# pierluigiferrari/ssd_keras

Hardware: AMD Instinct MI355X
Metric: images/sec SSD300 fwd+decode @batch32 (higher is better)
Workload: dtype f32 (decode, threshold, TF-style f32 NMS, top-k); bf16 conv backbone; 1 GPU; SSD300 VGG-16 inference (mode='inference': forward + DecodeDetections), 21 classes, batch 32 per GPU, conf 0.01 / NMS 0.45 / top-200, random-init weights, synthetic 300x300x3 uint8-range images; per_gpu_batch=32, global_batch=32, conv_dtype=bf16, parallelism=replicas x1, launch=hip_graph (forward + DecodeDetections captured once, replayed per step), decode_stream=same stream; DecodeDetections reads the head outputs directly (no y_pred in HBM)

## Files before the change

ssd_keras_amd/csrc/ssdhip_decode.hip:

```cpp
#include <hip/hip_runtime.h>
#include <stdint.h>
#include <stdlib.h>

#include "ssdhip.h"
#include "ssdhip_math.h"
#include "ssdhip_tile.h"
#include "ssdhip_heads.h"
#include "ssdhip_decode64.h"

#ifdef SSDHIP_PROFILE
__device__ unsigned long long g_prof[64];
#define PROF_DECL long long _pt = clock64(); long long _pa[12] = {0, 0, 0, 0, 0, 0, 0, 0, 0, 0, 0, 0};
#define PROF_MARK(i) { const long long _t = clock64(); _pa[i] += _t - _pt; _pt = _t; }
#define PROF_FLUSH(base) if (threadIdx.x == 0) { for (int _i = 0; _i < 12; ++_i) if (_pa[_i]) atomicAdd(&g_prof[(base) + _i], (unsigned long long)_pa[_i]); }
extern "C" int ssdhip_profile_read(unsigned long long* host_out, int reset) {
    if (hipMemcpyFromSymbol(host_out, HIP_SYMBOL(g_prof), sizeof(g_prof)) != hipSuccess) return -1;
    if (reset) { unsigned long long z[64] = {0}; if (hipMemcpyToSymbol(HIP_SYMBOL(g_prof), z, sizeof(z)) != hipSuccess) return -1; }
    return 0;
}
#else
#define PROF_DECL
#define PROF_MARK(i)
#define PROF_FLUSH(base)
#endif

namespace ssdhip {

constexpr int IDX_BITS = 20;
constexpr u32 IDX_MASK = (1u << IDX_BITS) - 1u;
constexpr int DIGIT_BITS = 13;
constexpr int NBINS = 1 << DIGIT_BITS;
constexpr int NMS_BIN_SHIFT = 14;
constexpr int NMS_NBINS = 4096;
#ifndef SSDHIP_MAX_CHUNK
#define SSDHIP_MAX_CHUNK 512
#endif
#ifndef SSDHIP_NMS_MINWAVES
#define SSDHIP_NMS_MINWAVES 3
#endif
constexpr int MAX_CHUNK = SSDHIP_MAX_CHUNK;
constexpr int KEPT_LDS = 256;
constexpr int KC_KEYS = 9216;
constexpr int TOPK_SORT_MAX = 4096;

struct DecodeParams {
    int B, N, C, L, G;
    int class_agnostic, semantics, coords, border;
    int thr_inclusive;
    float thr_eff;
    u32 thr_key;
    int iou_f32;
    int fast_ok;
    int px_f32;
    int no_nms;
    float filter_kE;
    double iou_thresh, img_w, img_h;
    int top_k, cap, cap_store, out_rows, sorted;
    int no_dma;
};

template <int SHIFT, int NB>
__device__ __forceinline__ int bin_of(u32 skey, u32 thr_key) {
    const u32 v = skey >> SHIFT, base = thr_key >> SHIFT;
    if (v <= base) return 0;
    const u32 d = v - base;
    return d > (u32)(NB - 1) ? NB - 1 : (int)d;
}

template <int SEM>
__device__ __forceinline__ float decode_center(float off, float var, float a_wh, float a_c) {
    if (SEM == SSDHIP_SEM_KERAS) return (off * var) * a_wh + a_c;
    if (SEM == SSDHIP_SEM_DEBUG) return (off * a_wh) * var + a_c;
    return off * (var * a_wh) + a_c;
}

__device__ __forceinline__ void scan_tile_body(const float* tile, int* wave_cnt, const DecodeParams& p, const int b, const int a0,
                                               const int na, float4* __restrict__ boxes, u64* __restrict__ cand,
                                               int* __restrict__ cand_count, unsigned short* __restrict__ cls_out) {
    const int TA = blockDim.x;
    const int L = p.L;
    const int tid = threadIdx.x;
    const int lane = tid & 63, wave = tid >> 6, nwaves = TA >> 6;
    PROF_DECL
    PROF_MARK(0)

    const bool active = tid < na;
    const float* row = tile + (size_t)tid * L;
    const int C = p.C;

    int fast_cls = 0;
    float fast_conf = 0.f;
    if (active) {
        const float o0 = row[C], o1 = row[C + 1], o2 = row[C + 2], o3 = row[C + 3];
        const float a_0 = row[C + 4], a_1 = row[C + 5], a_2 = row[C + 6], a_3 = row[C + 7];
        const float v0 = row[C + 8], v1 = row[C + 9], v2 = row[C + 10], v3 = row[C + 11];
        float4 box;
        if (p.coords == SSDHIP_CENTROIDS) {
            float cx, cy;
            if (p.semantics == SSDHIP_SEM_KERAS) {
                cx = decode_center<SSDHIP_SEM_KERAS>(o0, v0, a_2, a_0);
                cy = decode_center<SSDHIP_SEM_KERAS>(o1, v1, a_3, a_1);
            } else if (p.semantics == SSDHIP_SEM_DEBUG) {
                cx = decode_center<SSDHIP_SEM_DEBUG>(o0, v0, a_2, a_0);
                cy = decode_center<SSDHIP_SEM_DEBUG>(o1, v1, a_3, a_1);
            } else {
                cx = decode_center<SSDHIP_SEM_NUMPY>(o0, v0, a_2, a_0);
                cy = decode_center<SSDHIP_SEM_NUMPY>(o1, v1, a_3, a_1);
            }
            const float w = det_expf(o2 * v2) * a_2;
            const float h = det_expf(o3 * v3) * a_3;
            const float hw = w / 2.0f, hh = h / 2.0f;
            box = make_float4(cx - hw, cy - hh, cx + hw, cy + hh);
        } else if (p.coords == SSDHIP_MINMAX) {
            const float aw = a_1 - a_0, ah = a_3 - a_2;
            const float t0 = (o0 * v0) * aw + a_0, t1 = (o1 * v1) * aw + a_1;
            const float t2 = (o2 * v2) * ah + a_2, t3 = (o3 * v3) * ah + a_3;
            box = make_float4(t0, t2, t1, t3);
        } else {
            const float aw = a_2 - a_0, ah = a_3 - a_1;
            box = make_float4((o0 * v0) * aw + a_0, (o1 * v1) * ah + a_1, (o2 * v2) * aw + a_2, (o3 * v3) * ah + a_3);
        }
        boxes[(size_t)b * p.N + a0 + tid] = box;
        if (p.class_agnostic) {
            float best = row[0];
            int bi = 0;
            for (int c = 1; c < C; ++c) {
                const float s = row[c];
                if (s > best) { best = s; bi = c; }
            }
            for (int c = 0; c < C; ++c) if (row[c] != row[c]) { best = row[c]; bi = c; break; }
            fast_cls = bi;
            fast_conf = best;
            cls_out[(size_t)b * p.N + a0 + tid] = (unsigned short)bi;
        }
    }
    PROF_MARK(1)

    const int G = p.G;
    const float t = p.thr_eff;
    const bool incl = p.thr_inclusive != 0;
    const bool fast_pred = active && (fast_cls != 0) && (incl ? (fast_conf >= t) : (fast_conf > t));
    for (int gb = 0; gb < G; gb += 64) {
        const int ng = min(64, G - gb);
        int mycnt = 0;
        if (p.class_agnostic) {
            mycnt = __popcll(__ballot(fast_pred));
        } else {
            const float* sc = row + gb + 1;
            for (int j0 = 0; j0 < ng; j0 += 8) {
                float s8[8];
#pragma unroll
                for (int u = 0; u < 8; ++u) s8[u] = sc[min(j0 + u, ng - 1)];
#pragma unroll
                for (int u = 0; u < 8; ++u) {
                    const bool pr = active && (j0 + u < ng) && (incl ? (s8[u] >= t) : (s8[u] > t));
                    const int cnt = __popcll(__ballot(pr));
                    mycnt = lane == j0 + u ? cnt : mycnt;
                }
            }
        }
        if (lane < ng) wave_cnt[wave * G + gb + lane] = mycnt;
    }
    __syncthreads();
    PROF_MARK(2)
    for (int g = tid; g < G; g += TA) {
        int tot = 0;
        for (int w = 0; w < nwaves; ++w) tot += wave_cnt[w * G + g];
        int base = 0;
        if (tot) base = atomicAdd(&cand_count[b * G + g], tot);
        for (int w = 0; w < nwaves; ++w) {
            const int c = wave_cnt[w * G + g];
            wave_cnt[w * G + g] = base;
            base += c;
        }
    }
    __syncthreads();
    PROF_MARK(3)
    const u32 inv_idx = IDX_MASK - (u32)(a0 + tid);
    for (int gb = 0; gb < G; gb += 64) {
        const int ng = min(64, G - gb);
        const int mybase = lane < ng ? wave_cnt[wave * G + gb + lane] : 0;
        const float* sc = row + gb + 1;
        for (int j0 = 0; j0 < ng; j0 += 8) {
            float s8[8];
#pragma unroll
            for (int u = 0; u < 8; ++u) s8[u] = p.class_agnostic ? fast_conf : sc[min(j0 + u, ng - 1)];
#pragma unroll
            for (int u = 0; u < 8; ++u) {
                const int j = j0 + u;
                const float s = s8[u];
                const bool pr = (j < ng) && (p.class_agnostic ? fast_pred : (active && (incl ? (s >= t) : (s > t))));
                const u64 m = __ballot(pr);
                if (m == 0) continue;
                const int base_j = __builtin_amdgcn_readlane(mybase, j);
                if (pr) {
                    const int slot = base_j + (int)__builtin_amdgcn_mbcnt_hi((u32)(m >> 32), __builtin_amdgcn_mbcnt_lo((u32)m, 0u));
                    cand[((size_t)b * G + gb + j) * p.N + slot] = ((u64)float_key(s) << IDX_BITS) | inv_idx;
                }
            }
        }
    }
    PROF_MARK(4)
    PROF_FLUSH(16)
}

__global__ __launch_bounds__(256) void scan_kernel(const float* __restrict__ y, DecodeParams p,
                                                   float4* __restrict__ boxes, u64* __restrict__ cand,
                                                   int* __restrict__ cand_count, unsigned short* __restrict__ cls_out) {
    extern __shared__ __attribute__((aligned(16))) unsigned char smem_raw[];
    const int TA = blockDim.x;
    const int b = blockIdx.y;
    const int a0 = blockIdx.x * TA;
    const int na = min(TA, p.N - a0);
    const float* tile;
    const size_t total_bytes = (size_t)gridDim.y * p.N * (size_t)p.L * sizeof(float);
    if (!((uintptr_t)y & 15) && !(((size_t)p.N * p.L) & 3) && !((TA * p.L) & 3) && total_bytes < 0x7fffff00ull && !(TA & 63) && !p.no_dma) {
        const int lane = threadIdx.x & 63, wave = __builtin_amdgcn_readfirstlane((int)threadIdx.x >> 6);
        const u32 lds0 = (u32)(uintptr_t)(__attribute__((address_space(3))) unsigned char*)smem_raw;
        const i32x4 rs = tile_rsrc(y, (u32)total_bytes);
        const u32 off = (u32)(((size_t)b * p.N + a0) * (size_t)p.L * sizeof(float));
        const int nch = (na * p.L + 3) >> 2;
        for (int q0 = wave * 64; q0 < nch; q0 += TA) {
            const int q = q0 + lane;
            tile_dma16(q < nch ? off + (u32)q * 16u : TILE_OOB, rs, lds0 + (u32)q0 * 16u);
        }
        asm volatile("s_waitcnt vmcnt(0)" ::: "memory");
        tile = reinterpret_cast<const float*>(smem_raw);
    } else {
        tile = tile_copy_f32(reinterpret_cast<float*>(smem_raw), y + ((size_t)b * p.N + a0) * (size_t)p.L, na * p.L, threadIdx.x, TA);
    }
    int* wave_cnt = reinterpret_cast<int*>(smem_raw + (((size_t)TA * p.L + 4) * sizeof(float) + 15) / 16 * 16);
    __syncthreads();
    scan_tile_body(tile, wave_cnt, p, b, a0, na, boxes, cand, cand_count, cls_out);
}

constexpr int SW_WAVES = 4, SW_CW = 32, SW_PITCH = SW_CW + 1;
__global__ __launch_bounds__(SW_WAVES * 64) void scan_wide_kernel(const float* __restrict__ y, DecodeParams p, float4* __restrict__ boxes,
                                                                  u64* __restrict__ cand, int* __restrict__ cand_count) {
    __shared__ float win_all[SW_WAVES][64 * SW_PITCH];
    const int tid = threadIdx.x, lane = tid & 63, wave = tid >> 6;
    const int b = blockIdx.y;
    const int a0 = ((int)blockIdx.x * SW_WAVES + wave) * 64;
    if (a0 >= p.N) return;
    const int na = min(64, p.N - a0);
    float* win = win_all[wave];
    const int L = p.L, C = p.C, G = p.G;
    const float* src = y + ((size_t)b * p.N + a0) * (size_t)L;
    const float t = p.thr_eff;
    const bool incl = p.thr_inclusive != 0;
    const bool active = lane < na;
    const u32 inv_idx = IDX_MASK - (u32)(a0 + lane);
    const int nwin = (L + SW_CW - 1) / SW_CW;
    for (int wi = nwin - 1; wi >= 0; --wi) {
        const int c_hi = L - (nwin - 1 - wi) * SW_CW, c_lo = max(0, c_hi - SW_CW), cw = c_hi - c_lo;
        {
            const int c = lane & 31, rh = lane >> 5;
#pragma unroll
            for (int r0 = 0; r0 < 64; r0 += 16) {
                float v[8];
#pragma unroll
                for (int u = 0; u < 8; ++u) {
                    const int r = r0 + 2 * u + rh;
                    v[u] = (r < na && c < cw) ? src[(size_t)r * L + c_lo + c] : 0.f;
                }
#pragma unroll
                for (int u = 0; u < 8; ++u) win[(r0 + 2 * u + rh) * SW_PITCH + c] = v[u];
            }
        }
        __builtin_amdgcn_fence(__ATOMIC_RELEASE, "workgroup");
        __builtin_amdgcn_wave_barrier();
        const float* row = win + lane * SW_PITCH;
        if (wi == nwin - 1 && active) {
            const float* q = row + (cw - 12);
            const float o0 = q[0], o1 = q[1], o2 = q[2], o3 = q[3];
            const float a_0 = q[4], a_1 = q[5], a_2 = q[6], a_3 = q[7];
            const float v0 = q[8], v1 = q[9], v2 = q[10], v3 = q[11];
            float4 box;
            if (p.coords == SSDHIP_CENTROIDS) {
                float cx, cy;
                if (p.semantics == SSDHIP_SEM_KERAS) {
                    cx = decode_center<SSDHIP_SEM_KERAS>(o0, v0, a_2, a_0);
                    cy = decode_center<SSDHIP_SEM_KERAS>(o1, v1, a_3, a_1);
                } else if (p.semantics == SSDHIP_SEM_DEBUG) {
                    cx = decode_center<SSDHIP_SEM_DEBUG>(o0, v0, a_2, a_0);
                    cy = decode_center<SSDHIP_SEM_DEBUG>(o1, v1, a_3, a_1);
                } else {
                    cx = decode_center<SSDHIP_SEM_NUMPY>(o0, v0, a_2, a_0);
                    cy = decode_center<SSDHIP_SEM_NUMPY>(o1, v1, a_3, a_1);
                }
                const float w = det_expf(o2 * v2) * a_2;
                const float h = det_expf(o3 * v3) * a_3;
                const float hw = w / 2.0f, hh = h / 2.0f;
                box = make_float4(cx - hw, cy - hh, cx + hw, cy + hh);
            } else if (p.coords == SSDHIP_MINMAX) {
                const float aw = a_1 - a_0, ah = a_3 - a_2;
                const float t0 = (o0 * v0) * aw + a_0, t1 = (o1 * v1) * aw + a_1;
                const float t2 = (o2 * v2) * ah + a_2, t3 = (o3 * v3) * ah + a_3;
                box = make_float4(t0, t2, t1, t3);
            } else {
                const float aw = a_2 - a_0, ah = a_3 - a_1;
                box = make_float4((o0 * v0) * aw + a_0, (o1 * v1) * ah + a_1, (o2 * v2) * aw + a_2, (o3 * v3) * ah + a_3);
            }
            boxes[(size_t)b * p.N + a0 + lane] = box;
        }
        const int k_lo = max(c_lo, 1), k_hi = min(c_hi, C), nk = k_hi - k_lo;
        if (nk > 0) {
            int mycnt = 0;
            for (int j = 0; j < nk; ++j) {
                const float sc = row[k_lo - c_lo + j];
                const bool pr = active && (incl ? (sc >= t) : (sc > t));
                const int cnt = __popcll(__ballot(pr));
                mycnt = lane == j ? cnt : mycnt;
            }
            int mybase = 0;
            if (lane < nk && mycnt) mybase = atomicAdd(&cand_count[b * G + (k_lo - 1) + lane], mycnt);
            for (int j = 0; j < nk; ++j) {
                const float sc = row[k_lo - c_lo + j];
                const bool pr = active && (incl ? (sc >= t) : (sc > t));
                const u64 m = __ballot(pr);
                if (m == 0) continue;
                const int base_j = __builtin_amdgcn_readlane(mybase, j);
                if (pr) {
                    const int slot = base_j + (int)__builtin_amdgcn_mbcnt_hi((u32)(m >> 32), __builtin_amdgcn_mbcnt_lo((u32)m, 0u));
                    cand[((size_t)b * G + (k_lo - 1) + j) * p.N + slot] = ((u64)float_key(sc) << IDX_BITS) | inv_idx;
                }
            }
        }
        __builtin_amdgcn_fence(__ATOMIC_ACQUIRE, "workgroup");
        __builtin_amdgcn_wave_barrier();
    }
}

__global__ __launch_bounds__(256) void scan_heads_kernel(HeadParams hp, const float* __restrict__ anchors_var, DecodeParams p,
                                                         float4* __restrict__ boxes, u64* __restrict__ cand,
                                                         int* __restrict__ cand_count, unsigned short* __restrict__ cls_out) {
    extern __shared__ __attribute__((aligned(16))) unsigned char smem_raw[];
    const int b = blockIdx.y;
    int l, a0, na;
    head_tile_of(hp, (int)blockIdx.x, l, a0, na);
    float* rows = reinterpret_cast<float*>(smem_raw);
    bf16_t* cl = reinterpret_cast<bf16_t*>(smem_raw + (size_t)hp.TA * p.L * sizeof(float));
    int* wave_cnt = reinterpret_cast<int*>(smem_raw + (head_tile_lds(hp.TA, p.C) + 15) / 16 * 16);
    head_build_rows(hp, anchors_var, l, b, a0, na, rows, cl, threadIdx.x, blockDim.x);
    scan_tile_body(rows, wave_cnt, p, b, hp.anchor_off[l] + a0, na, boxes, cand, cand_count, cls_out);
}

template <int KEY_BITS, int DB, int T, typename KeyF>
__device__ u64 block_select_kth(KeyF key_at, int n, u64 upper, bool has_upper, int k, u32* hist, int* red) {
    const int tid = threadIdx.x;
    constexpr int NB = 1 << DB;
    u64 prefix = 0, pmask = 0;
    constexpr int NPASS = (KEY_BITS + DB - 1) / DB;
    for (int pass = 0; pass < NPASS; ++pass) {
        const int shift = (NPASS - 1 - pass) * DB;
        for (int i = tid; i < NB; i += T) hist[i] = 0;
        __syncthreads();
        for (int i = tid; i < n; i += T) {
            const u64 key = key_at(i);
            if (has_upper && !(key < upper)) continue;
            if ((key & pmask) != prefix) continue;
            atomicAdd(&hist[(u32)(key >> shift) & (NB - 1)], 1u);
        }
        __syncthreads();
        block_find_digit<NB / T>(hist, k, red, red + 256);
        const int d = red[256];
        k -= red[257];
        prefix |= (u64)d << shift;
        pmask |= (u64)(NB - 1) << shift;
        __syncthreads();
    }
    return prefix;
}

template <typename F>
struct __attribute__((aligned(16))) NBox {
    F x0, y0, x1, y1, area;
    u32 idx;
    u32 ok;
};

template <typename F>
__device__ __forceinline__ bool is_finite(F v) { return v - v == (F)0; }

template <typename F>
__device__ __forceinline__ NBox<F> make_nbox(const float4 bx, u32 idx, F W, F H, F d, bool px_f32) {
    NBox<F> r;
    if (px_f32) {
        r.x0 = (F)(float)((double)bx.x * (double)W); r.y0 = (F)(float)((double)bx.y * (double)H);
        r.x1 = (F)(float)((double)bx.z * (double)W); r.y1 = (F)(float)((double)bx.w * (double)H);
    } else {
        r.x0 = (F)bx.x * W; r.y0 = (F)bx.y * H; r.x1 = (F)bx.z * W; r.y1 = (F)bx.w * H;
    }
    r.area = box_area<F>(r.x0, r.y0, r.x1, r.y1, d);
    r.idx = idx;
    r.ok = (is_finite(r.x0) && is_finite(r.y0) && is_finite(r.x1) && is_finite(r.y1) && is_finite(r.area)) ? 1u : 0u;
    return r;
}

__device__ __forceinline__ int nms_test(const NBox<double>& a, const NBox<double>& b, double thr, int fast_ok) {
    const double ix0 = fmax(a.x0, b.x0), iy0 = fmax(a.y0, b.y0);
    const double ix1 = fmin(a.x1, b.x1), iy1 = fmin(a.y1, b.y1);
    const double iw = fmax(ix1 - ix0, 0.0), ih = fmax(iy1 - iy0, 0.0);
    const double inter = iw * ih;
    const double uni = (a.area + b.area) - inter;
    const double tu = thr * uni;
    const double r = fma(-thr, uni, inter);
    const bool fin = (a.ok & b.ok & (u32)fast_ok) != 0u;
    const bool zero = uni == 0.0 && inter == 0.0;
    const bool dec = uni > 0x1p-900 && fabs(r) > 0x1p-50 * tu;
    return fin ? (zero ? 1 : (dec ? (r > 0.0 ? 1 : 0) : 2)) : 2;
}
__device__ __forceinline__ int nms_test(const NBox<float>& a, const NBox<float>& b, float thr, int) {
    const PxBox<float> pa = {a.x0, a.y0, a.x1, a.y1, a.area}, pb = {b.x0, b.y0, b.x1, b.y1, b.area};
    return (iou_px<float>(pa, pb) <= thr) ? 0 : 1;
}

template <typename F>
__device__ __forceinline__ bool exact_suppresses(const NBox<F>& a, const NBox<F>& b, F thr) {
    const PxBox<F> pa = {a.x0, a.y0, a.x1, a.y1, a.area}, pb = {b.x0, b.y0, b.x1, b.y1, b.area};
    return !(iou_px<F>(pa, pb) <= thr);
}

enum { POL_NUMPY64 = 0, POL_NUMPY32 = 1, POL_TF32 = 2 };

struct __attribute__((aligned(16))) FBox {
    float x0, y0, x1, y1;
    float area;
// ... 857 lines not shown
    const float* anchors_var;
    int tiles;
};

static int decode_run(const HeadSource* heads, int stages, const void* y_pred, int in_dtype, int B, int N, int C,
                      double conf_thresh, double iou_thresh, int top_k, int nms_cap,
                      int class_agnostic, int semantics,
                      int coords, int normalize_coords, double img_height, double img_width,
                      int border_pixels,
                      void* out, int out_dtype, int out_rows, int* out_count, int* out_anchor_idx,
                      void* ws, size_t ws_bytes, void* stream_) {
    hipStream_t stream = static_cast<hipStream_t>(stream_);
    if ((!y_pred && !heads) || !out || !out_count || B <= 0 || N <= 0 || C < 2 || out_rows <= 0) return SSDHIP_E_BADARG;
    if (in_dtype != SSDHIP_F32 && in_dtype != SSDHIP_F64) return SSDHIP_E_BADARG;
    if (out_dtype != SSDHIP_F32 && out_dtype != SSDHIP_F64) return SSDHIP_E_BADARG;
    if (N > (1 << IDX_BITS) || C > 1025) return SSDHIP_E_BADARG;
    if (coords < 0 || coords > 2 || border_pixels < 0 || border_pixels > 2) return SSDHIP_E_BADARG;
    if (semantics < 0 || semantics > 2) return SSDHIP_E_BADARG;
    if (in_dtype == SSDHIP_F64) {
        if (heads || !y_pred) return SSDHIP_E_BADARG;
        return decode64_run(stages, static_cast<const double*>(y_pred), B, N, C, conf_thresh, iou_thresh, top_k, nms_cap,
                            class_agnostic, semantics, coords, normalize_coords, img_height, img_width, border_pixels, out, out_dtype,
                            out_rows, out_count, out_anchor_idx, ws, ws_bytes, stream);
    }
    if (semantics == SSDHIP_SEM_KERAS && coords != SSDHIP_CENTROIDS) return SSDHIP_E_BADARG;
    const int sorted = semantics == SSDHIP_SEM_KERAS;
    if (sorted && (top_k <= 0 || top_k > TOPK_SORT_MAX)) return SSDHIP_E_BADARG;
    const DecodeWs lay = decode_ws_layout(B, N, C, top_k, nms_cap, class_agnostic);
    if (!ws || ws_bytes < lay.total) return SSDHIP_E_WORKSPACE;

    DecodeParams p;
    p.B = B; p.N = N; p.C = C; p.L = C + 12; p.G = class_agnostic ? 1 : C - 1;
    p.no_dma = 0;
    p.class_agnostic = class_agnostic ? 1 : 0;
    p.semantics = semantics; p.coords = coords; p.border = border_pixels;
    p.iou_f32 = (semantics != SSDHIP_SEM_KERAS && coords == SSDHIP_CORNERS) ? 1 : 0;
    p.thr_inclusive = (class_agnostic && semantics != SSDHIP_SEM_KERAS) ? 1 : 0;
    {
        const bool cmp_f32 = (semantics == SSDHIP_SEM_KERAS) || p.iou_f32;
        float te = (float)conf_thresh;
        if (!cmp_f32 && conf_thresh == conf_thresh && te - te == 0.f) {
            if (!p.thr_inclusive && (double)te > conf_thresh) te = nextafterf(te, -INFINITY);
            if (p.thr_inclusive && (double)te < conf_thresh) te = nextafterf(te, INFINITY);
        }
        p.thr_eff = te;
        union { float f; unsigned u; } cv;
        cv.f = te;
        const unsigned key = (cv.u & 0x80000000u) ? ~cv.u : (cv.u | 0x80000000u);
        p.thr_key = key;
    }
    p.iou_thresh = iou_thresh;
    p.img_w = normalize_coords ? img_width : 1.0;
    p.img_h = normalize_coords ? img_height : 1.0;
    p.fast_ok = (iou_thresh > 0.0 && iou_thresh < 1e300) ? 1 : 0;
    if (semantics == SSDHIP_SEM_KERAS) p.fast_ok = ((float)iou_thresh >= 1e-30f && (float)iou_thresh < 1e30f) ? 1 : 0;
    p.px_f32 = (semantics == SSDHIP_SEM_KERAS) ? 1 : 0;
    p.no_nms = (iou_thresh == (double)INFINITY) ? 1 : 0;
    p.filter_kE = (iou_thresh > 0.0 && iou_thresh <= 16.0) ? (float)((16.0 + 40.0 * iou_thresh) * 0x1p-24 * 1.001) : INFINITY;
    if (p.px_f32 && ((double)(float)p.img_w != p.img_w || (double)(float)p.img_h != p.img_h)) return SSDHIP_E_BADARG;
    p.top_k = top_k; p.cap = nms_cap; p.cap_store = cap_store_for(N, top_k, nms_cap);
    p.out_rows = out_rows; p.sorted = sorted;

    unsigned char* base = static_cast<unsigned char*>(ws);
    float4* boxes = reinterpret_cast<float4*>(base + lay.boxes);
    int* cand_count = reinterpret_cast<int*>(base + lay.cand_count);
    int* kept_count = reinterpret_cast<int*>(base + lay.kept_count);
    unsigned short* cls_map = reinterpret_cast<unsigned short*>(base + lay.cls);
    u64* cand = reinterpret_cast<u64*>(base + lay.cand);
    u64* kept = reinterpret_cast<u64*>(base + lay.kept);

    if (stages & 1) {
    if (zero_async(cand_count, (size_t)B * p.G * sizeof(int), stream) != hipSuccess) return SSDHIP_E_LAUNCH;

    int TA = 256;
    while (TA > 64 && (size_t)TA * p.L * sizeof(float) > 24 * 1024) TA >>= 1;
    size_t k3_lds = align_up(((size_t)TA * p.L + 4) * sizeof(float), 16) + (size_t)(TA / 64) * p.G * sizeof(int);
    k3_lds = k3_lds > align_up((size_t)TA * p.L * sizeof(float), 1024) ? k3_lds : align_up((size_t)TA * p.L * sizeof(float), 1024);
    { const char* e = getenv("SSDHIP_SCAN_DMA"); p.no_dma = (e && e[0] == '0') ? 1 : 0; }
    if (k3_lds > 160 * 1024) return SSDHIP_E_BADARG;
    if (heads) {
        const int HT = heads->hp->TA;
        const size_t lds = (head_tile_lds(HT, C) + 15) / 16 * 16 + (size_t)((HT + 63) / 64) * p.G * sizeof(int);
        if (lds > 160 * 1024) return SSDHIP_E_BADARG;
        hipLaunchKernelGGL(scan_heads_kernel, dim3(heads->tiles, B), dim3(HT < 64 ? 64 : HT), lds, stream, *heads->hp,
                           heads->anchors_var, p, boxes, cand, cand_count, cls_map);
    } else if (p.L > 64 && !p.class_agnostic) {
        dim3 g3((N + SW_WAVES * 64 - 1) / (SW_WAVES * 64), B);
        hipLaunchKernelGGL(scan_wide_kernel, g3, dim3(SW_WAVES * 64), 0, stream, static_cast<const float*>(y_pred), p, boxes, cand, cand_count);
    } else {
        dim3 g3((N + TA - 1) / TA, B);
        hipLaunchKernelGGL(scan_kernel, g3, dim3(TA), k3_lds, stream, static_cast<const float*>(y_pred), p, boxes, cand,
                           cand_count, cls_map);
    }
    if (hipGetLastError() != hipSuccess) return SSDHIP_E_LAUNCH;
    }

    if (stages & 2) {
    const int work = B * p.G;
    const int g4 = ((work + 7) / 8) * 8;
    const int* order = nullptr;
    static const int nms_env = []() { const char* e = getenv("SSDHIP_NMS_T"); return e ? atoi(e) : 0; }();
    const int nms_t = nms_env ? nms_env : (semantics == SSDHIP_SEM_KERAS ? 512 : 256);
#define SSDHIP_LAUNCH_NMS(POL)                                                                                                            \
    do {                                                                                                                                  \
        if (nms_t >= 512) {                                                                                                               \
            hipLaunchKernelGGL((nms_kernel<POL, 512, false>), dim3(g4), dim3(512), 0, stream, p, boxes, cand, cand_count, order, kept, kept_count, 0); \
            hipLaunchKernelGGL((nms_kernel<POL, 512, true>), dim3(g4), dim3(512), 0, stream, p, boxes, cand, cand_count, order, kept, kept_count, 1); \
        } else {                                                                                                                          \
            hipLaunchKernelGGL((nms_kernel<POL, 256, true>), dim3(g4), dim3(256), 0, stream, p, boxes, cand, cand_count, order, kept, kept_count, 0); \
        }                                                                                                                                 \
    } while (0)
    if (semantics == SSDHIP_SEM_KERAS) SSDHIP_LAUNCH_NMS(POL_TF32);
    else if (p.iou_f32) SSDHIP_LAUNCH_NMS(POL_NUMPY32);
    else SSDHIP_LAUNCH_NMS(POL_NUMPY64);
#undef SSDHIP_LAUNCH_NMS
    if (hipGetLastError() != hipSuccess) return SSDHIP_E_LAUNCH;
    }

    if (stages & 4) {
    size_t sort_cap = 4096;
    while (sort_cap < (size_t)p.G * (size_t)p.cap_store && sort_cap < 16384) sort_cap <<= 1;
    const size_t k5_lds = sort_cap * sizeof(u64) + align_up((size_t)(p.G + 1) * sizeof(int), 16);
    const void* fn = out_dtype == SSDHIP_F32 ? reinterpret_cast<const void*>(topk_kernel<float>) : reinterpret_cast<const void*>(topk_kernel<double>);
    if (k5_lds > 48 * 1024 && hipFuncSetAttribute(fn, hipFuncAttributeMaxDynamicSharedMemorySize, (int)k5_lds) != hipSuccess) return SSDHIP_E_LAUNCH;
    if (out_dtype == SSDHIP_F32)
        hipLaunchKernelGGL(topk_kernel<float>, dim3(B), dim3(TOPK_THREADS), k5_lds, stream, p, boxes, kept, kept_count, cls_map,
                           static_cast<float*>(out), out_count, out_anchor_idx, (int)sort_cap);
    else
        hipLaunchKernelGGL(topk_kernel<double>, dim3(B), dim3(TOPK_THREADS), k5_lds, stream, p, boxes, kept, kept_count, cls_map,
                           static_cast<double*>(out), out_count, out_anchor_idx, (int)sort_cap);
    if (hipGetLastError() != hipSuccess) return SSDHIP_E_LAUNCH;
    }
    return SSDHIP_OK;
}

extern "C" int ssdhip_decode_detections(const void* y_pred, int in_dtype, int B, int N, int C,
                                        double conf_thresh, double iou_thresh, int top_k, int nms_cap,
                                        int class_agnostic, int semantics,
                                        int coords, int normalize_coords, double img_height, double img_width,
                                        int border_pixels,
                                        void* out, int out_dtype, int out_rows, int* out_count, int* out_anchor_idx,
                                        void* ws, size_t ws_bytes, void* stream) {
    return decode_run(nullptr, 7, y_pred, in_dtype, B, N, C, conf_thresh, iou_thresh, top_k, nms_cap, class_agnostic, semantics, coords,
                      normalize_coords, img_height, img_width, border_pixels, out, out_dtype, out_rows, out_count,
                      out_anchor_idx, ws, ws_bytes, stream);
}

extern "C" int ssdhip_decode_stages(int stages, const void* y_pred, int in_dtype, int B, int N, int C,
                                    double conf_thresh, double iou_thresh, int top_k, int nms_cap,
                                    int class_agnostic, int semantics,
                                    int coords, int normalize_coords, double img_height, double img_width,
                                    int border_pixels,
                                    void* out, int out_dtype, int out_rows, int* out_count, int* out_anchor_idx,
                                    void* ws, size_t ws_bytes, void* stream) {
    if (stages <= 0 || stages > 7) return SSDHIP_E_BADARG;
    return decode_run(nullptr, stages, y_pred, in_dtype, B, N, C, conf_thresh, iou_thresh, top_k, nms_cap, class_agnostic, semantics,
                      coords, normalize_coords, img_height, img_width, border_pixels, out, out_dtype, out_rows, out_count,
                      out_anchor_idx, ws, ws_bytes, stream);
}

static int decode_from_heads_any(int src_f32, int n_layers, const void* const* conf_h, const void* const* loc_h,
                                 const void* const* conf_bias_h, const void* const* loc_bias_h, const int* n_anchors_h,
                                 const int* n_boxes_h, const int* conf_stride_h, const int* loc_stride_h, const float* anchors_var,
                                 int B, int N, int C, double conf_thresh, double iou_thresh, int top_k, int nms_cap, int class_agnostic,
                                 int semantics, int coords, int normalize_coords, double img_height, double img_width, int border_pixels,
                                 void* out, int out_dtype, int out_rows, int* out_count, int* out_anchor_idx, void* ws, size_t ws_bytes,
// ... 44 lines not shown
```

ssd_keras_amd/csrc/ssdhip_heads.h:

```cpp
#pragma once
#include <hip/hip_runtime.h>
#include <stdint.h>
#include <stdlib.h>

#include "ssdhip.h"
#include "ssdhip_math.h"
#include "ssdhip_bf16.h"
#include "ssdhip_tile.h"

namespace ssdhip {

constexpr int MAX_PRED_LAYERS = 8;
struct HeadParams {
    const bf16_t* conf[MAX_PRED_LAYERS];
    const bf16_t* loc[MAX_PRED_LAYERS];
    const bf16_t* conf_bias[MAX_PRED_LAYERS];
    const bf16_t* loc_bias[MAX_PRED_LAYERS];
    int n_anchors[MAX_PRED_LAYERS];
    int n_boxes[MAX_PRED_LAYERS];
    int conf_stride[MAX_PRED_LAYERS];
    int loc_stride[MAX_PRED_LAYERS];
    int tile_start[MAX_PRED_LAYERS + 1];
    int anchor_off[MAX_PRED_LAYERS];
    int n_layers, N, C, TA;
// ... 160 lines not shown
                    for (int u = 0; u < 4; ++u) r[c + u] = e[u] / sum;
                }
                for (; c < C; ++c) r[c] = r[c] / sum;
                const bf16_t* lsrc = prow + nb * C + box * 4;
                const bf16_t* lb = bs + nb * C + box * 4;
#pragma unroll
                for (int k = 0; k < 4; ++k) r[C + k] = has_lb ? bf16_float(bf16_bits(bf16_float(lsrc[k]) + bf16_float(lb[k]))) : bf16_float(lsrc[k]);
                if (av16 && a == tid) {
                    r[C + 4] = av0.x; r[C + 5] = av0.y; r[C + 6] = av0.z; r[C + 7] = av0.w;
                    r[C + 8] = av1.x; r[C + 9] = av1.y; r[C + 10] = av1.z; r[C + 11] = av1.w;
                } else {
                    const float* av = anchors_var + (size_t)(hp.anchor_off[l] + a0 + a) * 8;
                    for (int k = 0; k < 8; ++k) r[C + 4 + k] = av[k];
                }
            }
            __syncthreads();
            return;
        }
    }
    if (hp.conf_stride[l] == nb * C && hp.loc_stride[l] == nb * 4) {
        const bf16_t* csrc = hp.conf[l] + ((size_t)b * hp.n_anchors[l] + a0) * C;
        const bf16_t* lsrc = hp.loc[l] + ((size_t)b * hp.n_anchors[l] + a0) * 4;
        for (int i = tid; i < na * C; i += nthreads) cl[i] = csrc[i];
        for (int i = tid; i < na * 4; i += nthreads) ll[i] = lsrc[i];
    } else {
        const size_t px0 = (size_t)b * (hp.n_anchors[l] / nb);
        {
            const int step_a = nthreads / C, step_c = nthreads - step_a * C;
            int c = tid % C;
            const int ga0 = a0 + tid / C;
            int pix = ga0 / nb, box = ga0 - pix * nb;
            const bf16_t* src = hp.conf[l] + px0 * hp.conf_stride[l];
            const int cs = hp.conf_stride[l];
            const int q0 = step_a / nb, r0 = step_a - q0 * nb, q1 = (step_a + 1) / nb, r1 = step_a + 1 - q1 * nb;
            for (int i = tid; i < na * C; i += nthreads) {
                cl[i] = src[(size_t)pix * cs + box * C + c];
                c += step_c;
                const bool carry = c >= C;
                c -= carry ? C : 0;
                box += carry ? r1 : r0;
                pix += carry ? q1 : q0;
                if (box >= nb) { box -= nb; ++pix; }
            }
        }
        {
            const int step_a = nthreads >> 2;
            const int k = tid & 3;
            const int ga0 = a0 + (tid >> 2);
            int pix = ga0 / nb, box = ga0 - pix * nb;
            const bf16_t* src = hp.loc[l] + px0 * hp.loc_stride[l];
            const int ls = hp.loc_stride[l];
            const int q0 = step_a / nb, r0 = step_a - q0 * nb;
            for (int i = tid; i < na * 4; i += nthreads) {
                ll[i] = src[(size_t)pix * ls + box * 4 + k];
                box += r0;
                pix += q0;
                if (box >= nb) { box -= nb; ++pix; }
            }
        }
    }
    __syncthreads();
    for (int a = tid; a < na; a += nthreads) {
        const int box = (a0 + a) % nb;
        float* r = rows + (size_t)a * L;
        const bf16_t* cb = hp.conf_bias[l] ? hp.conf_bias[l] + box * C : nullptr;
        float mx = -INFINITY;
        for (int c = 0; c < C; ++c) {
            const float v = cb ? bf16_float(bf16_bits(bf16_float(cl[a * C + c]) + bf16_float(cb[c]))) : bf16_float(cl[a * C + c]);
            r[c] = v;
            mx = fmaxf(mx, v);
        }
        double acc = 0.0;
        for (int c = 0; c < C; ++c) { const float e = expf(r[c] - mx); r[c] = e; acc += (double)e; }
        const float sum = (float)acc;
        for (int c = 0; c < C; ++c) r[c] = r[c] / sum;
        const bf16_t* lb = hp.loc_bias[l] ? hp.loc_bias[l] + box * 4 : nullptr;
        for (int k = 0; k < 4; ++k) r[C + k] = lb ? bf16_float(bf16_bits(bf16_float(ll[a * 4 + k]) + bf16_float(lb[k]))) : bf16_float(ll[a * 4 + k]);
        const float* av = anchors_var + (size_t)(hp.anchor_off[l] + a0 + a) * 8;
        for (int k = 0; k < 8; ++k) r[C + 4 + k] = av[k];
    }
    __syncthreads();
}

static inline int head_fill_params(HeadParams& hp, int n_layers, const void* const* conf_h, const void* const* loc_h,
                                   const void* const* conf_bias_h, const void* const* loc_bias_h, const int* n_anchors_h,
                                   const int* n_boxes_h, const int* conf_stride_h, const int* loc_stride_h, int N, int C,
                                   size_t max_lds, int* tiles_out, int src_f32 = 0) {
    if (n_layers <= 0 || n_layers > MAX_PRED_LAYERS || !conf_h || !loc_h || !n_anchors_h || !n_boxes_h || N <= 0 || C < 2 || C > 1024)
        return SSDHIP_E_BADARG;
    const int TA = head_tile_anchors(C, max_lds);
    hp.n_layers = n_layers; hp.N = N; hp.C = C; hp.TA = TA; hp.src_f32 = src_f32 ? 1 : 0;
    { const char* e = getenv("SSDHIP_HEADS_DMA"); hp.row_dma = !(e && e[0] == '0'); }
    if (src_f32 && (conf_bias_h || loc_bias_h)) {
        for (int l = 0; l < n_layers; ++l)
            if ((conf_bias_h && conf_bias_h[l]) || (loc_bias_h && loc_bias_h[l])) return SSDHIP_E_BADARG;
    }
    int off = 0, tiles = 0;
    for (int l = 0; l < MAX_PRED_LAYERS; ++l) {
        const bool on = l < n_layers;
        hp.conf[l] = on ? static_cast<const bf16_t*>(conf_h[l]) : nullptr;
        hp.loc[l] = on ? static_cast<const bf16_t*>(loc_h[l]) : nullptr;
        hp.conf_bias[l] = (on && conf_bias_h) ? static_cast<const bf16_t*>(conf_bias_h[l]) : nullptr;
        hp.loc_bias[l] = (on && loc_bias_h) ? static_cast<const bf16_t*>(loc_bias_h[l]) : nullptr;
        hp.n_anchors[l] = on ? n_anchors_h[l] : 0;
        hp.n_boxes[l] = on ? n_boxes_h[l] : 1;
        hp.conf_stride[l] = on ? (conf_stride_h ? conf_stride_h[l] : n_boxes_h[l] * C) : 0;
        hp.loc_stride[l] = on ? (loc_stride_h ? loc_stride_h[l] : n_boxes_h[l] * 4) : 0;
        hp.tile_start[l] = tiles;
        hp.anchor_off[l] = off;
        if (on) {
            if (!hp.conf[l] || !hp.loc[l] || hp.n_anchors[l] <= 0 || hp.n_boxes[l] <= 0 || hp.n_anchors[l] % hp.n_boxes[l]) return SSDHIP_E_BADARG;
            if (hp.conf_stride[l] < hp.n_boxes[l] * C || hp.loc_stride[l] < hp.n_boxes[l] * 4) return SSDHIP_E_BADARG;
            off += hp.n_anchors[l];
            tiles += (hp.n_anchors[l] + TA - 1) / TA;
        }
    }
    hp.tile_start[MAX_PRED_LAYERS] = tiles;
    if (off != N) return SSDHIP_E_BADARG;
    *tiles_out = tiles;
    return SSDHIP_OK;
}

}
```

Measured before the change: 16590 images/sec.

## Keep decoded head rows in registers with a C=21 specialized scan kernel

Adds a scan_heads_rows_kernel<21> that DMA-stages the bf16 head outputs into LDS, then has each thread build its own softmaxed score, loc and anchor row directly in registers instead of writing full f32 rows to LDS. The scan body is templated on a row accessor so the class loops are fully unrolled at compile time, with one lane per class and no per-8-class batching. This is meant to cut LDS traffic and LDS footprint, which should allow more resident blocks (launch bounds 256, 5). The cost is much higher register pressure from a 33-float row per thread and a specialised path gated on C==21 and DMA-compatible layouts.

```diff
diff --git a/ssd_keras_amd/csrc/ssdhip_decode.hip b/ssd_keras_amd/csrc/ssdhip_decode.hip
--- a/ssd_keras_amd/csrc/ssdhip_decode.hip
+++ b/ssd_keras_amd/csrc/ssdhip_decode.hip
@@ -74,19 +74,31 @@
     return off * (var * a_wh) + a_c;
 }
 
-__device__ __forceinline__ void scan_tile_body(const float* tile, int* wave_cnt, const DecodeParams& p, const int b, const int a0,
+struct LdsRow {
+    static constexpr int CT = 0;
+    const float* r;
+    __device__ __forceinline__ float operator[](int i) const { return r[i]; }
+};
+template <int C_>
+struct RegRow {
+    static constexpr int CT = C_;
+    float r[C_ + 12];
+    __device__ __forceinline__ float operator[](int i) const { return r[i]; }
+};
+
+template <typename Row>
+__device__ __forceinline__ void scan_tile_body(const Row& row, int* wave_cnt, const DecodeParams& p, const int b, const int a0,
                                                const int na, float4* __restrict__ boxes, u64* __restrict__ cand,
                                                int* __restrict__ cand_count, unsigned short* __restrict__ cls_out) {
+    constexpr int CT = Row::CT;
     const int TA = blockDim.x;
-    const int L = p.L;
     const int tid = threadIdx.x;
     const int lane = tid & 63, wave = tid >> 6, nwaves = TA >> 6;
     PROF_DECL
     PROF_MARK(0)
 
     const bool active = tid < na;
-    const float* row = tile + (size_t)tid * L;
-    const int C = p.C;
+    const int C = CT ? CT : p.C;
 
     int fast_cls = 0;
     float fast_conf = 0.f;
@@ -124,11 +136,21 @@
         if (p.class_agnostic) {
             float best = row[0];
             int bi = 0;
+            if constexpr (CT > 0) {
+#pragma unroll
+                for (int c = 1; c < CT; ++c) {
+                    const float s = row[c];
+                    if (s > best) { best = s; bi = c; }
+                }
+#pragma unroll
+                for (int c = CT - 1; c >= 0; --c) if (row[c] != row[c]) { best = row[c]; bi = c; }
+            } else {
             for (int c = 1; c < C; ++c) {
                 const float s = row[c];
                 if (s > best) { best = s; bi = c; }
             }
             for (int c = 0; c < C; ++c) if (row[c] != row[c]) { best = row[c]; bi = c; break; }
+            }
             fast_cls = bi;
             fast_conf = best;
             cls_out[(size_t)b * p.N + a0 + tid] = (unsigned short)bi;
@@ -140,13 +162,29 @@
     const float t = p.thr_eff;
     const bool incl = p.thr_inclusive != 0;
     const bool fast_pred = active && (fast_cls != 0) && (incl ? (fast_conf >= t) : (fast_conf > t));
+    if constexpr (CT > 0) {
+        static_assert(CT - 1 <= 64, "one lane per class");
+        int mycnt = 0;
+        if (p.class_agnostic) {
+            mycnt = __popcll(__ballot(fast_pred));
+        } else {
+#pragma unroll
+            for (int j = 0; j < CT - 1; ++j) {
+                const float s = row[j + 1];
+                const bool pr = active && (incl ? (s >= t) : (s > t));
+                const int cnt = __popcll(__ballot(pr));
+                mycnt = lane == j ? cnt : mycnt;
+            }
+        }
+        if (lane < G) wave_cnt[wave * G + lane] = mycnt;
+    } else
     for (int gb = 0; gb < G; gb += 64) {
         const int ng = min(64, G - gb);
         int mycnt = 0;
         if (p.class_agnostic) {
             mycnt = __popcll(__ballot(fast_pred));
         } else {
-            const float* sc = row + gb + 1;
+            const float* sc = row.r + gb + 1;
             for (int j0 = 0; j0 < ng; j0 += 8) {
                 float s8[8];
 #pragma unroll
@@ -177,10 +215,34 @@
     __syncthreads();
     PROF_MARK(3)
     const u32 inv_idx = IDX_MASK - (u32)(a0 + tid);
+    if constexpr (CT > 0) {
+        const int mybase = lane < G ? wave_cnt[wave * G + lane] : 0;
+        if (p.class_agnostic) {
+            const u64 m = __ballot(fast_pred);
+            const int base_0 = __builtin_amdgcn_readlane(mybase, 0);
+            if (fast_pred) {
+                const int slot = base_0 + (int)__builtin_amdgcn_mbcnt_hi((u32)(m >> 32), __builtin_amdgcn_mbcnt_lo((u32)m, 0u));
+                cand[(size_t)b * G * p.N + slot] = ((u64)float_key(fast_conf) << IDX_BITS) | inv_idx;
+            }
+        } else {
+#pragma unroll
+            for (int j = 0; j < CT - 1; ++j) {
+                const float s = row[j + 1];
+                const bool pr = active && (incl ? (s >= t) : (s > t));
+                const u64 m = __ballot(pr);
+                if (m == 0) continue;
+                const int base_j = __builtin_amdgcn_readlane(mybase, j);
+                if (pr) {
+                    const int slot = base_j + (int)__builtin_amdgcn_mbcnt_hi((u32)(m >> 32), __builtin_amdgcn_mbcnt_lo((u32)m, 0u));
+                    cand[((size_t)b * G + j) * p.N + slot] = ((u64)float_key(s) << IDX_BITS) | inv_idx;
+                }
+            }
+        }
+    } else
     for (int gb = 0; gb < G; gb += 64) {
         const int ng = min(64, G - gb);
         const int mybase = lane < ng ? wave_cnt[wave * G + gb + lane] : 0;
-        const float* sc = row + gb + 1;
+        const float* sc = row.r + gb + 1;
         for (int j0 = 0; j0 < ng; j0 += 8) {
             float s8[8];
 #pragma unroll
@@ -231,7 +293,7 @@
     }
     int* wave_cnt = reinterpret_cast<int*>(smem_raw + (((size_t)TA * p.L + 4) * sizeof(float) + 15) / 16 * 16);
     __syncthreads();
-    scan_tile_body(tile, wave_cnt, p, b, a0, na, boxes, cand, cand_count, cls_out);
+    scan_tile_body(LdsRow{tile + (size_t)threadIdx.x * p.L}, wave_cnt, p, b, a0, na, boxes, cand, cand_count, cls_out);
 }
 
 constexpr int SW_WAVES = 4, SW_CW = 32, SW_PITCH = SW_CW + 1;
@@ -342,7 +404,21 @@
     bf16_t* cl = reinterpret_cast<bf16_t*>(smem_raw + (size_t)hp.TA * p.L * sizeof(float));
     int* wave_cnt = reinterpret_cast<int*>(smem_raw + (head_tile_lds(hp.TA, p.C) + 15) / 16 * 16);
     head_build_rows(hp, anchors_var, l, b, a0, na, rows, cl, threadIdx.x, blockDim.x);
-    scan_tile_body(rows, wave_cnt, p, b, hp.anchor_off[l] + a0, na, boxes, cand, cand_count, cls_out);
+    scan_tile_body(LdsRow{rows + (size_t)threadIdx.x * p.L}, wave_cnt, p, b, hp.anchor_off[l] + a0, na, boxes, cand, cand_count, cls_out);
+}
+
+template <int C>
+__global__ __launch_bounds__(256, 5) void scan_heads_rows_kernel(HeadParams hp, const float* __restrict__ anchors_var, DecodeParams p,
+                                                                 float4* __restrict__ boxes, u64* __restrict__ cand,
+                                                                 int* __restrict__ cand_count, unsigned short* __restrict__ cls_out) {
+    extern __shared__ __attribute__((aligned(16))) unsigned char smem_raw[];
+    const int b = blockIdx.y;
+    int l, a0, na;
+    head_tile_of(hp, (int)blockIdx.x, l, a0, na);
+    int* wave_cnt = reinterpret_cast<int*>(smem_raw + (head_stage_bytes(hp.TA, C) + 15) / 16 * 16);
+    RegRow<C> row;
+    head_row_regs<C>(hp, anchors_var, l, b, a0, na, smem_raw, threadIdx.x, blockDim.x, row.r);
+    scan_tile_body(row, wave_cnt, p, b, hp.anchor_off[l] + a0, na, boxes, cand, cand_count, cls_out);
 }
 
 template <int KEY_BITS, int DB, int T, typename KeyF>
@@ -1366,6 +1442,13 @@
         const int HT = heads->hp->TA;
         const size_t lds = (head_tile_lds(HT, C) + 15) / 16 * 16 + (size_t)((HT + 63) / 64) * p.G * sizeof(int);
         if (lds > 160 * 1024) return SSDHIP_E_BADARG;
+        const char* rows_env = getenv("SSDHIP_SCAN_ROWS");
+        const bool rows_lds = rows_env && rows_env[0] == 'l' && rows_env[1] == 'd' && rows_env[2] == 's' && !rows_env[3];
+        if (!rows_lds && C == 21 && HT == 256 && heads->hp->C == C && head_rows_all_dma(*heads->hp, B, HT, heads->anchors_var)) {
+            const size_t rlds = (head_stage_bytes(HT, C) + 15) / 16 * 16 + (size_t)(HT / 64) * p.G * sizeof(int);
+            hipLaunchKernelGGL(scan_heads_rows_kernel<21>, dim3(heads->tiles, B), dim3(HT), rlds, stream, *heads->hp, heads->anchors_var,
+                               p, boxes, cand, cand_count, cls_map);
+        } else
         hipLaunchKernelGGL(scan_heads_kernel, dim3(heads->tiles, B), dim3(HT < 64 ? 64 : HT), lds, stream, *heads->hp,
                            heads->anchors_var, p, boxes, cand, cand_count, cls_map);
     } else if (p.L > 64 && !p.class_agnostic) {
diff --git a/ssd_keras_amd/csrc/ssdhip_heads.h b/ssd_keras_amd/csrc/ssdhip_heads.h
--- a/ssd_keras_amd/csrc/ssdhip_heads.h
+++ b/ssd_keras_amd/csrc/ssdhip_heads.h
@@ -266,6 +266,83 @@
     __syncthreads();
 }
 
+template <int C>
+__device__ __forceinline__ void head_row_regs(const HeadParams& hp, const float* __restrict__ anchors_var, int l, int b, int a0, int na,
+                                              unsigned char* st, int tid, int nthreads, float (&r)[C + 12]) {
+    const int nb = hp.n_boxes[l];
+    const int stride = hp.conf_stride[l];
+    const int U = nb * (C + 4) * 2, cpr = (U + 15) >> 4, pitch = cpr * 16;
+    const int pix0 = a0 / nb, npx = (a0 + na - 1) / nb - pix0 + 1, nchunks = npx * cpr;
+    const size_t dma_area = (size_t)((nchunks + 63) >> 6) * 1024;
+    const size_t npix_l = (size_t)(hp.n_anchors[l] / nb);
+    const size_t src_bytes = (size_t)gridDim.y * npix_l * (size_t)stride * 2;
+    const u32 lds0 = (u32)(uintptr_t)(__attribute__((address_space(3))) unsigned char*)st;
+    const i32x4 rs = tile_rsrc(hp.conf[l], (u32)src_bytes);
+    const int lane = tid & 63, wave = __builtin_amdgcn_readfirstlane(tid >> 6);
+    const u32 row0 = (u32)(((size_t)b * npix_l + pix0) * (size_t)stride * 2);
+    for (int q0 = wave * 64; q0 < nchunks; q0 += nthreads) {
+        const int q = q0 + lane, rr = q / cpr, j = q - rr * cpr;
+        tile_dma16(q < nchunks ? row0 + (u32)rr * (u32)(stride * 2) + (u32)j * 16u : TILE_OOB, rs, lds0 + (u32)q0 * 16u);
+    }
+    bf16_t* bs = reinterpret_cast<bf16_t*>(st + dma_area);
+    const bool has_cb = hp.conf_bias[l] != nullptr, has_lb = hp.loc_bias[l] != nullptr;
+    if (has_cb) for (int i = tid; i < nb * C; i += nthreads) bs[i] = hp.conf_bias[l][i];
+    if (has_lb) for (int i = tid; i < nb * 4; i += nthreads) bs[nb * C + i] = hp.loc_bias[l][i];
+    float4 av0 = make_float4(0.f, 0.f, 0.f, 0.f), av1 = av0;
+    if (tid < na) {
+        const float4* avp = reinterpret_cast<const float4*>(anchors_var + (size_t)(hp.anchor_off[l] + a0 + tid) * 8);
+        av0 = avp[0]; av1 = avp[1];
+    }
+    asm volatile("s_waitcnt vmcnt(0)" ::: "memory");
+    __syncthreads();
+#pragma unroll
+    for (int k = 0; k < C + 12; ++k) r[k] = 0.f;
+    if (tid < na) {
+        const int ga = a0 + tid, pix = ga / nb, box = ga - pix * nb;
+        const bf16_t* prow = reinterpret_cast<const bf16_t*>(st + (size_t)(pix - pix0) * pitch);
+        const bf16_t* src = prow + box * C;
+        const bf16_t* cb = bs + box * C;
+        float mx = -INFINITY;
+#pragma unroll
+        for (int c = 0; c < C; ++c) {
+            const float x = bf16_float(src[c]);
+            r[c] = has_cb ? bf16_float(bf16_bits(x + bf16_float(cb[c]))) : x;
+            mx = fmaxf(mx, r[c]);
+        }
+        double acc = 0.0;
+#pragma unroll
+        for (int c = 0; c < C; ++c) { r[c] = expf(r[c] - mx); acc += (double)r[c]; }
+        const float sum = (float)acc;
+#pragma unroll
+        for (int c = 0; c < C; ++c) r[c] = r[c] / sum;
+        const bf16_t* lsrc = prow + nb * C + box * 4;
+        const bf16_t* lb = bs + nb * C + box * 4;
+#pragma unroll
+        for (int k = 0; k < 4; ++k) r[C + k] = has_lb ? bf16_float(bf16_bits(bf16_float(lsrc[k]) + bf16_float(lb[k]))) : bf16_float(lsrc[k]);
+        r[C + 4] = av0.x; r[C + 5] = av0.y; r[C + 6] = av0.z; r[C + 7] = av0.w;
+        r[C + 8] = av1.x; r[C + 9] = av1.y; r[C + 10] = av1.z; r[C + 11] = av1.w;
+    }
+}
+
+static inline bool head_rows_all_dma(const HeadParams& hp, int B, int nthreads, const float* anchors_var) {
+    if (!hp.row_dma || hp.src_f32 || (nthreads & 63) || nthreads != hp.TA || ((uintptr_t)anchors_var & 15)) return false;
+    const int C = hp.C, TA = hp.TA;
+    for (int l = 0; l < hp.n_layers; ++l) {
+        const int nb = hp.n_boxes[l], stride = hp.conf_stride[l];
+        const int U = nb * (C + 4) * 2, cpr = (U + 15) >> 4, pitch = cpr * 16;
+        const size_t src_bytes = (size_t)B * (size_t)(hp.n_anchors[l] / nb) * (size_t)stride * 2;
+        if (hp.loc[l] != hp.conf[l] + (size_t)nb * C || hp.loc_stride[l] != stride || (stride & 7) || stride * 2 < pitch ||
+            ((uintptr_t)hp.conf[l] & 15) || src_bytes >= 0x7fffff00ull)
+            return false;
+        for (int a0 = 0; a0 < hp.n_anchors[l]; a0 += TA) {
+            const int na = hp.n_anchors[l] - a0 < TA ? hp.n_anchors[l] - a0 : TA;
+            const int pix0 = a0 / nb, npx = (a0 + na - 1) / nb - pix0 + 1, nchunks = npx * cpr;
+            if ((size_t)((nchunks + 63) >> 6) * 1024 + (size_t)U > head_stage_bytes(TA, C)) return false;
+        }
+    }
+    return true;
+}
+
 static inline int head_fill_params(HeadParams& hp, int n_layers, const void* const* conf_h, const void* const* loc_h,
                                    const void* const* conf_bias_h, const void* const* loc_bias_h, const int* n_anchors_h,
                                    const int* n_boxes_h, const int* conf_stride_h, const int* loc_stride_h, int N, int C,
```

Result: faster. 16770 images/sec (median of 6 runs) (+1.0%).
